# SiftScience/kafka-assigner

Measured on AMD Instinct MI355X. Metric: assignment scenarios/sec at 100k partitions x 1k brokers RF=3, higher is better.
Workload: dtype int32

## Files before the change

kafka-assigner_amd/csrc/kas_order_relax.h:

```cpp
#pragma once

namespace kas {

#define KAS_RELAX_F0_ONE 0x1u
#define KAS_RELAX_F1_ONE 0x10000u
#define KAS_RELAX_F1_MASK 0xffff0000u
#define KAS_RELAX_PAD_WORD 0xfff0fff0u
#define KAS_RELAX_PICK_BITS 0x00010001u

KAS_DEV uint32_t relax_row_word(uint32_t w0, uint32_t w1) { return (KAS_RELAX_F0_ONE << w0) | (KAS_RELAX_F1_ONE << w1); }

#define KAS_RELAX_MAXP 12
struct RelaxPairs {
  uint32_t* slot;
  const uint32_t* row[KAS_RELAX_MAXP];
  uint32_t cell[KAS_RELAX_MAXP];
};

struct RelaxTopic {
  int32_t idx2, idx3;
  uint32_t vp3;
  uint32_t ord2;
};

// ... 11 lines not shown
  }
  return t;
}

KAS_DEV int32_t relax_eval_generic(const uint32_t (&x)[3], const bool (&valid)[3], const int32_t (&rank)[3], int32_t Lp,
                                   const RelaxTopic& t) {
  const int32_t idx_m0 = Lp == 3 ? t.idx3 : (Lp == 2 ? t.idx2 : 0);
  uint32_t best = 0xffffffffu;
#pragma unroll
  for (int k = 0; k < 3; ++k) {
    int32_t vp = idx_m0 + rank[k];
    vp -= vp >= Lp ? Lp : 0;
    const uint32_t key = ((x[k] & 0xffffu) << 8) | ((uint32_t)vp << 2) | (uint32_t)k;
    best = (valid[k] && key < best) ? key : best;
  }
  const int32_t w0 = Lp >= 1 ? (int32_t)(best & 3u) : 0;
  best = 0xffffffffu;
#pragma unroll
  for (int k = 0; k < 3; ++k) {
    const int32_t ord = (Lp == 3 && t.idx2) ? 2 - rank[k] : rank[k];
    const uint32_t key = ((x[k] >> 16) << 8) | ((uint32_t)ord << 2) | (uint32_t)k;
    best = (valid[k] && k != w0 && key < best) ? key : best;
  }
  const int32_t w1 = Lp >= 2 ? (int32_t)(best & 3u) : 0;
  return w0 | (w1 << 2);
}

template <int NP, class Word>
KAS_DEV void relax_exchange(Word* slot, Word* const (&padr)[NP], Word (&padd)[NP], const Word (&nadd)[NP], bool undo) {
  constexpr bool WORD64 = sizeof(Word) == 8;
  if (undo) {
#pragma unroll
    for (int t = 0; t < NP; ++t) {
      if constexpr (WORD64) kasw::lds_sub_u64(padr[t], padd[t]);
      else kasw::lds_sub_u32(padr[t], padd[t]);
    }
  }
  kasw::lockstep();
  Word got[NP];
#pragma unroll
  for (int t = 0; t < NP; ++t) {
    if constexpr (WORD64) got[t] = kasw::lds_add_rtn_u64(padr[t], nadd[t]);
    else got[t] = kasw::lds_add_rtn_u32(padr[t], nadd[t]);
    kasw::lockstep();
    padd[t] = nadd[t];
  }
#pragma unroll
  for (int t = 0; t < NP; ++t) slot[64 * t] = got[t];
  kasw::lockstep();
}

template <int NP>
KAS_DEV void relax_pairs(const RelaxPairs& pp, uint32_t* const (&padr)[NP], uint32_t (&padd)[NP], bool undo) {
  kasw::lockstep();
  uint32_t nadd[NP];
#pragma unroll
  for (int t = 0; t < NP; ++t) nadd[t] = (*pp.row[t] >> pp.cell[t]) & KAS_RELAX_PICK_BITS;
  relax_exchange<NP, uint32_t>(pp.slot, padr, padd, nadd, undo);
}

struct RelaxTags { uint32_t t0[3], t1[3]; };

KAS_DEV RelaxTags relax_tags(const uint32_t (&c)[3], const uint32_t* tagtab) {
  const uint32_t oidx = ((c[0] - c[1]) >> 31) | (((c[0] - c[2]) >> 31) << 1) | (((c[1] - c[2]) >> 31) << 2);
  const uint32_t tw = tagtab[oidx];
  RelaxTags g;
#pragma unroll
  for (int q = 0; q < 3; ++q) { g.t0[q] = (tw >> (4 * q)) & 15u; g.t1[q] = (tw >> (12 + 4 * q)) & 15u; }
  return g;
}

KAS_DEV RelaxTags relax_tags_sorted(const RelaxTopic& t) {
  RelaxTags g;
#pragma unroll
  for (int q = 0; q < 3; ++q) {
    g.t0[q] = ((t.vp3 >> (4 * q)) & 0xcu) | (uint32_t)q;
    g.t1[q] = ((t.ord2 >> (4 * q)) & 0xcu) | (uint32_t)q;
  }
  return g;
}

#ifndef KAS_M32_SORTED_TAGS
#define KAS_M32_SORTED_TAGS(M32) (M32)
#endif
KAS_DEV int32_t relax_eval3(const uint32_t (&x)[3], const RelaxTags& g) {
  const uint32_t k00 = (x[0] << 16) | g.t0[0], k01 = (x[1] << 16) | g.t0[1], k02 = (x[2] << 16) | g.t0[2];
  const uint32_t kmin = k00 < k01 ? (k00 < k02 ? k00 : k02) : (k01 < k02 ? k01 : k02);
  const uint32_t w0 = kmin & 3u;
  const uint32_t k10 = (x[0] & KAS_RELAX_F1_MASK) | g.t1[0], k11 = (x[1] & KAS_RELAX_F1_MASK) | g.t1[1],
                 k12 = (x[2] & KAS_RELAX_F1_MASK) | g.t1[2];
  const uint32_t lo = w0 == 0u ? k11 : k10, hi = w0 == 2u ? k11 : k12;
  const uint32_t w1 = (lo < hi ? lo : hi) & 3u;
  return (int32_t)(w0 | (w1 << 2));
}

template <class Raw>
KAS_DEV void relax_list3(const Raw& raw, int32_t oc, uint32_t (&l)[3], uint32_t* cnt2 = nullptr) {
  const uint32_t w0 = (uint32_t)oc & 3u, w1 = ((uint32_t)oc >> 2) & 3u, w2 = 3u - w0 - w1;
  l[0] = kasw::perm_bytes(raw.w[1], raw.w[0], 0x0c0c0100u + w0 * 0x0202u);
  l[1] = kasw::perm_bytes(raw.w[1], raw.w[0], 0x0c0c0100u + w1 * 0x0202u);
  l[2] = kasw::perm_bytes(raw.w[1], raw.w[0], 0x0c0c0100u + w2 * 0x0202u);
  if (cnt2) kasw::lds_add_u32(cnt2 + l[2], 1u);
}

template <int NB>
struct RelaxPend {
  uint32_t id[NB][3];
  int32_t p;
  int32_t n;
};

template <int W, bool FULLW, bool M32 = false>
KAS_DEV void mid_request(MidRaw<W>& r, const uint16_t* mid, int32_t ow, int32_t p) {
  if constexpr (M32) {
    kasw::gload_u32_async<0>(r.w[0], mid, (uint32_t)p * 4u);
  } else if constexpr (FULLW) {
    const uint32_t off = (uint32_t)p * (uint32_t)(2 * mid_width_of<W>());
    kasw::gload_u32_async<0>(r.w[0], mid, off);
    if constexpr (W == 3) kasw::gload_u16_async<4>(r.w[1], mid, off);
  } else {
    const uint32_t off = (uint32_t)p * (uint32_t)(2 * mid_width(ow));
#pragma unroll
    for (int k = 0; k < W; ++k) kasw::gload_u16_async<0>(r.w[k], mid, off + 2u * (uint32_t)(k < ow ? k : ow - 1));
  }
}
template <int W, bool FULLW, bool M32 = false>
KAS_DEV MidRaw<W> mid_take(const MidRaw<W>& r, int32_t ow, bool active) {
  MidRaw<W> o;
  if constexpr (M32) {
    o.w[0] = active ? r.w[0] : 0xffffffffu;
#pragma unroll
    for (int k = 1; k < W; ++k) o.w[k] = 0xffffffffu;
    return o;
  }
#pragma unroll
  for (int k = 0; k < W; ++k) o.w[k] = (active && (FULLW ? k < (W + 1) / 2 : k < ow)) ? r.w[k] : 0xffffffffu;
  return o;
}

template <int W, bool FULLW, bool M32>
KAS_DEV MidRaw<W> mid_view(const MidRaw<W>& t, int32_t ow) {
  if constexpr (M32) {
    static_assert(W == 3, "dword mid rows: lists 3 wide");
    MidRaw<W> o;
    uint32_t f[3];
    mid32_fields(t.w[0], f);
    if constexpr (FULLW) {
      o.w[0] = f[0] | (f[1] << 16);
      o.w[1] = f[2] | 0xffff0000u;
      o.w[2] = 0xffffffffu;
    } else {
#pragma unroll
      for (int k = 0; k < 3; ++k) o.w[k] = (k < ow && f[k] != KAS_M32_NONE) ? f[k] : 0xffffffffu;
    }
    return o;
  } else {
    return t;
  }
}

template <int NB, bool C16 = false>
KAS_DEV uint64_t relax_flush(RelaxPend<NB>& pend, int32_t* out, uint16_t* out16, uint32_t k) {
  uint64_t d = 0;
#pragma unroll
  for (int b = 0; b < NB; ++b) {
    if (b < pend.n) {
      RowW<3> o;
#pragma unroll
      for (int q = 0; q < 3; ++q) {
        o.v[q] = (int32_t)pend.id[b][q];
        d += kas_digest_cell(k, (uint32_t)(pend.p + 64 * b), (uint32_t)q, o.v[q]);
      }
#if !defined(KAS_TUNE_NO_ROW_STORES)
      if constexpr (C16) {
        uint16_t* row = out16 + (int64_t)(pend.p + 64 * b) * 3;
        store_u32_a2(row, (uint32_t)o.v[0] | ((uint32_t)o.v[1] << 16));
        row[2] = (uint16_t)o.v[2];
      } else {
        *reinterpret_cast<RowW<3>*>(out + (int64_t)(pend.p + 64 * b) * 3) = o;
      }
#endif
    }
  }
  pend.n = 0;
  return d;
// ... 101 lines not shown
  bool aborted = false;
  auto rows_final = [&](int32_t k, int32_t upto) -> bool {
    if constexpr (FS) {
      int32_t idle = 0;
      for (;;) {
        kasw::repoll();
        const uint64_t f = kasw::load_shared_u64_lds(&fs[0]), fk = kasw::load_shared_u64_lds(&fs[1]);
        const int32_t ft = (int32_t)(f >> 32), fr = (int32_t)(uint32_t)f;
        if (kasw::ballot(fk <= (uint64_t)(uint32_t)k) != 0ull) return false;
        if (kasw::ballot(ft > k || (ft == k && fr >= upto)) != 0ull) return true;
        if (watchdog_poll(reinterpret_cast<uint32_t*>(&fs[3]), false, idle)) { stuck = true; return false; }
      }
    }
    return true;
  };
  for (int32_t k = 0; k < sd.topic_count; ++k) {
    const int32_t ti = sd.topic_begin + k;
    if constexpr (FS) {
      if (!rows_final(k, 0)) { aborted = true; break; }
    }
    if (a.topic_results[ti].status != KAS_OK) continue;
    const kas_topic_desc td = a.topics[ti];
    const int32_t P = td.n_partitions, ow = td.out_width;
    if (P <= 0) continue;
    uint64_t dtop = 0;
    int32_t* out = C16 ? nullptr : a.out + td.out_off;
    uint16_t* out16 = C16 ? reinterpret_cast<uint16_t*>(a.out) + td.out_off : nullptr;
    const uint16_t* mid = C16 ? out16 : (M32 ? reinterpret_cast<const uint16_t*>(out + (int64_t)P * ow - P) : mid_base(out, P, ow));
    const RelaxTopic rt = relax_topic(td.name_hash);
    const RelaxTags gsorted = relax_tags_sorted(rt);
    constexpr uint32_t NONE_FROM = M32 ? KAS_M32_NONE : 0x8000u;
    const int32_t nt = (P + 63) >> 6;
    kasw::lockstep();
    if (lane < 8) {
      const int32_t ab = lane & 1, ac = (lane >> 1) & 1, bc = (lane >> 2) & 1;
      const int32_t rank[3] = {(1 - ab) + (1 - ac), ab + (1 - bc), ac + bc};
      uint32_t w = 0u;
#pragma unroll
      for (int q = 0; q < 3; ++q) {
        w |= (((rt.vp3 >> (4 * rank[q])) & 0xcu) | (uint32_t)q) << (4 * q);
        w |= (((rt.ord2 >> (4 * rank[q])) & 0xcu) | (uint32_t)q) << (12 + 4 * q);
      }
      tagtab[lane] = w;
    }
    kasw::lockstep();
    const uint16_t* umid = kasw::uniform_ptr(mid);
    const int32_t* uid = kasw::uniform_ptr(g_node_id);
    auto topic_rows = [&](auto fullw_tag) {
      constexpr bool FULLW = decltype(fullw_tag)::value;
      constexpr int NB = NBT;
      const int32_t vstride = verify_k > 0 ? (nt / verify_k > 0 ? nt / verify_k : 1) : 0;
      const int32_t voff = vstride > 0 ? s % vstride : 0;
      auto row_exists = [&](int32_t t) -> bool { return ((t << 6) + lane) < P; };
      auto request_tile = [&](MidRaw<W>& r, int32_t t) {
        const int32_t pn = (t << 6) + lane;
        mid_request<W, FULLW, M32>(r, umid, ow, pn < P ? pn : 0);
      };
      MidRaw<W> raw[NB], nx[NB];
      RelaxPend<NB> pend;
      pend.n = 0; pend.p = 0;
#pragma unroll
      for (int b = 0; b < NB; ++b) {
#pragma unroll
        for (int q = 0; q < W; ++q) { raw[b].w[q] = 0xffffffffu; nx[b].w[q] = 0xffffffffu; }
#pragma unroll
        for (int q = 0; q < 3; ++q) pend.id[b][q] = 0u;
      }
#pragma unroll
      for (int b = 0; b < NB; ++b) request_tile(nx[b], b);
      kasw::wait_loads();
#pragma unroll
      for (int b = 0; b < NB; ++b) {
#pragma unroll
        for (int q = 0; q < (M32 ? 1 : W); ++q) kasw::arrived(nx[b].w[q]);
        raw[b] = mid_take<W, FULLW, M32>(nx[b], ow, row_exists(b));
      }
#pragma unroll
      for (int b = 0; b < NB; ++b) request_tile(nx[b], NB + b);
      for (int32_t tile = 0; tile < nt;) {
        const int32_t p = (tile << 6) + lane;
        const bool active = p < P;
        const MidRaw<W> ra = mid_view<W, FULLW, M32>(raw[0], ow);
        uint32_t c[3];
        if constexpr (FULLW) {
          c[0] = ra.w[0] & 0xffffu; c[1] = ra.w[0] >> 16; c[2] = W == 3 ? (ra.w[1] & 0xffffu) : KAS_MID_NONE;
        } else {
#pragma unroll
          for (int q = 0; q < 3; ++q) c[q] = q < W ? (ra.w[q] & 0xffffu) : KAS_MID_NONE;
        }
        bool fast = false;
        int32_t step = 1;
        int32_t req_n = 0;
        uint32_t req_l[NB][3];
#pragma unroll
        for (int b = 0; b < NB; ++b)
#pragma unroll
          for (int q = 0; q < 3; ++q) req_l[b][q] = 0u;
        auto usual_step = [&](auto nr_tag) -> bool {
          constexpr int NR = decltype(nr_tag)::value, NP = 3 * NR;
          MidRaw<W> rv[NR];
          uint32_t cc[NR][3];
          rv[0] = ra;
#pragma unroll
          for (int q = 0; q < 3; ++q) cc[0][q] = c[q];
          bool short_row = false;
#pragma unroll
          for (int b = 1; b < NR; ++b) {
            rv[b] = mid_view<W, FULLW, M32>(raw[b], ow);
            cc[b][0] = rv[b].w[0] & 0xffffu; cc[b][1] = rv[b].w[0] >> 16; cc[b][2] = rv[b].w[1] & 0xffffu;
            short_row = short_row || (M32 ? cc[b][2] >= NONE_FROM : ((cc[b][0] | cc[b][1] | cc[b][2]) & 0x8000u) != 0u);
          }
          if constexpr (NR > 1) {
            if (kasw::ballot(short_row) != 0ull) return false;
          }
          n_tiles += NR;
          kasw::lockstep();
#pragma unroll
          for (int b = 0; b < NR; ++b)
#pragma unroll
            for (int q = 0; q < 3; ++q) mine[192 * b + q] = cc[b][q];
          kasw::lockstep();
          uint32_t* padr[NP];
          uint32_t padd[NP];
#pragma unroll
          for (int t = 0; t < NP; ++t) { padr[t] = cnt + pp.slot[64 * t]; padd[t] = 0u; }
          RelaxTags g[NR];
          uint32_t x[NR][3];
#pragma unroll
          for (int b = 0; b < NR; ++b) g[b] = KAS_M32_SORTED_TAGS(M32) ? gsorted : relax_tags(cc[b], tagtab);
#pragma unroll
          for (int b = 0; b < NR; ++b)
#pragma unroll
            for (int q = 0; q < 3; ++q) x[b][q] = cnt[cc[b][q]];
          kasw::lockstep();
          int32_t prev[NR];
#pragma unroll
          for (int b = 0; b < NR; ++b) prev[b] = -1;
#pragma nounroll
          for (int32_t it = 0;; ++it) {
            n_evals += NR;
            if (it > 64 * NR + 2) { stuck = true; break; }
            int32_t oc[NR];
            bool moved = false;
#pragma unroll
            for (int b = 0; b < NR; ++b) { oc[b] = relax_eval3(x[b], g[b]); moved = moved || oc[b] != prev[b]; }
            if (kasw::ballot(moved) == 0ull) break;
#pragma unroll
            for (int b = 0; b < NR; ++b) rbuf[64 * b + lane] = relax_row_word((uint32_t)oc[b] & 3u, (uint32_t)oc[b] >> 2);
            relax_pairs<NP>(pp, padr, padd, it > 0);
#pragma unroll
            for (int b = 0; b < NR; ++b) {
#pragma unroll
              for (int q = 0; q < 3; ++q) x[b][q] = mine[192 * b + q];
              prev[b] = oc[b];
            }
          }
          rows1 += 64u * NR; rows2 += 64u * NR;
          if constexpr (VERIFY) {
            bool sampled = false;
#pragma unroll
            for (int b = 0; b < NR; ++b) sampled = sampled || (vstride > 0 && ((tile + b) % vstride) == voff);
            if (sampled) {
              n_verified += NR;
#pragma unroll
              for (int t = 0; t < NP; ++t) kasw::lds_sub_u32(padr[t], padd[t]);
              kasw::lockstep();
#pragma unroll
              for (int b = 0; b < NR; ++b)
                if (relax_verify_rows(cnt, rv[b].w[0], rv[b].w[1], tagtab, prev[b]) != 0ull) unsound = true;
            }
          }
#pragma unroll
          for (int b = 0; b < NR; ++b) relax_list3(rv[b], prev[b] < 0 ? 4 : prev[b], req_l[b], cnt2);
          req_n = NR;
          step = NR;
          return true;
        };
        bool settled = false;
        if constexpr (W == 3) {
          if (FULLW && ((tile + 1) << 6) <= P)
            fast = M32 ? kasw::ballot(c[2] >= NONE_FROM) == 0ull
                       : kasw::ballot(((c[0] | c[1] | c[2]) & 0x8000u) != 0u) == 0ull;
          if constexpr (NBT > 1) {
            if (fast && ((tile + NBT) << 6) <= P) settled = usual_step(std::integral_constant<int, NBT>{});
          }
          if (!settled && fast) settled = usual_step(std::integral_constant<int, 1>{});
        }
        if (!settled) {
          n_tiles += 1;
          n_slow += 1;
          kasw::lockstep();
#pragma unroll
          for (int q = 0; q < 3; ++q) mine[q] = c[q];
          kasw::lockstep();
          if constexpr (M32) {
#pragma unroll
            for (int q = 0; q < 3; ++q) c[q] = c[q] >= NONE_FROM ? KAS_MID_NONE : c[q];
          }
          uint32_t* padr[3];
          uint32_t padd[3] = {0u, 0u, 0u};
#pragma unroll
          for (int t = 0; t < 3; ++t) {
            const uint32_t n = pp.slot[64 * t];
            padr[t] = cnt + (n < (uint32_t)nmax ? n : (uint32_t)nmax);
          }
          uint32_t x[3];
#pragma unroll
          for (int q = 0; q < 3; ++q) x[q] = cnt[c[q] < (uint32_t)nmax ? c[q] : (uint32_t)nmax];
          kasw::lockstep();
          bool valid[3];
          int32_t rank[3], Lp = 0;
#pragma unroll
          for (int q = 0; q < 3; ++q) { valid[q] = active && (c[q] & 0x8000u) == 0u; Lp += valid[q] ? 1 : 0; }
#pragma unroll
          for (int q = 0; q < 3; ++q) {
            rank[q] = 0;
#pragma unroll
            for (int j = 0; j < 3; ++j) rank[q] += (j != q && valid[j] && c[j] < c[q]) ? 1 : 0;
          }
          rows1 += (uint32_t)kasw::popc(kasw::ballot(Lp >= 1)); rows2 += (uint32_t)kasw::popc(kasw::ballot(Lp >= 2));
          int32_t oc_prev = -1;
          for (int32_t it = 0;; ++it) {
            n_evals += 1;
            if (it > 66) { stuck = true; break; }
            const int32_t oc = relax_eval_generic(x, valid, rank, Lp, rt);
            if (kasw::ballot(oc != oc_prev) == 0ull) break;
            const uint32_t w0 = (uint32_t)oc & 3u, w1 = ((uint32_t)oc >> 2) & 3u;
            rbuf[lane] = (Lp >= 1 ? KAS_RELAX_F0_ONE << w0 : 0u) | (Lp >= 2 ? KAS_RELAX_F1_ONE << w1 : 0u);
            relax_pairs<3>(pp, padr, padd, it > 0);
#pragma unroll
            for (int q = 0; q < 3; ++q) x[q] = mine[q];
            oc_prev = oc;
          }
          if (active && oc_prev >= 0) {
            const int32_t w0 = oc_prev & 3, w1 = (oc_prev >> 2) & 3, w2 = 3 - w0 - w1;
            const int32_t w[3] = {w0, w1, w2};
#pragma unroll
            for (int r = 0; r < W; ++r) {
              if (r < ow) {
                const uint32_t cell = w[r] == 0 ? c[0] : (w[r] == 1 ? c[1] : c[2]);
                const int32_t id = r < Lp ? (C16 ? (int32_t)cell : (LDSIDS ? (int32_t)idt[cell] : g_node_id[cell])) : -1;
                if constexpr (CTX) { if (r == 2 && r < Lp) kasw::lds_add_u32(cnt2 + cell, 1u); }
                if constexpr (C16) out16[(int64_t)p * ow + r] = (uint16_t)id;
                else out[(int64_t)p * ow + r] = id;
                if (r < Lp) dtop += kas_digest_cell((uint32_t)k, (uint32_t)p, (uint32_t)r, id);
              }
            }
          }
        }
        tile += step;
        kasw::wait_loads();
#pragma unroll
        for (int b = 0; b < NB; ++b) {
#pragma unroll
          for (int q = 0; q < (M32 ? 1 : W); ++q) kasw::arrived(nx[b].w[q]);
#pragma unroll
// ... 117 lines not shown
```

kafka-assigner_amd/csrc/kas_solver_body.h:

```cpp
#pragma once
#include <stdint.h>

#include <type_traits>

#include "kas_abi.h"
#include "kas_plan_math.h"
#include "kas_wave.h"

#ifdef KAS_FILL_COUNTERS
#define KAS_COUNT(x) do { (x) += 1; } while (0)
#define KAS_COUNTERS_ON 1
#else
#define KAS_COUNT(x) do { } while (0)
#define KAS_COUNTERS_ON 0
#endif

#ifndef KAS_SPIN_BOUND
#define KAS_SPIN_BOUND (1 << 25)
#endif
#ifndef KAS_WIDE_SPIN_BOUND
#define KAS_WIDE_SPIN_BOUND KAS_SPIN_BOUND
#endif
#ifndef KAS_SPIN_CHECK
#define KAS_SPIN_CHECK 4096
// ... 394 lines not shown
template <int W>
KAS_DEV bool full_rows_of(const TopicView& T) { return T.cw == W && T.ow == W && T.len_arr == nullptr; }

#ifndef KAS_TILES_AHEAD
#define KAS_TILES_AHEAD 4
#endif
template <int W, bool FULL, bool C16, typename Body>
KAS_DEV void for_tiles_impl(const TopicView& T, int32_t tile0, int32_t stride, int32_t t_end, Body body) {
  constexpr int D = KAS_TILES_AHEAD;
  const int lane = kasw::lane();
  int32_t nx[D][W], nlen[D];
#pragma unroll
  for (int d = 0; d < D; ++d) load_row<W, FULL, C16>(T, ((tile0 + d * stride) << 6) + lane, nx[d], nlen[d]);
  for (int32_t tile = tile0; tile < t_end; tile += stride * D) {
    int32_t ids[D][W], len[D];
#pragma unroll
    for (int d = 0; d < D; ++d) {
#pragma unroll
      for (int r = 0; r < W; ++r) ids[d][r] = nx[d][r];
      len[d] = nlen[d];
    }
#pragma unroll
    for (int d = 0; d < D; ++d)
      load_row<W, FULL, C16>(T, ((tile + (D + d) * stride) << 6) + lane, nx[d], nlen[d]);
#pragma unroll
    for (int d = 0; d < D; ++d) {
      const int32_t t = tile + d * stride;
      if (t < t_end) body(t, ids[d], len[d]);
    }
  }
}

template <int W, bool FULL, bool C16, typename Body>
KAS_DEV void for_tile_batches_impl(const TopicView& T, int32_t tile0, int32_t stride, int32_t t_end, Body body) {
  constexpr int D = KAS_TILES_AHEAD;
  const int lane = kasw::lane();
  int32_t nx[D][W], nlen[D];
#pragma unroll
  for (int d = 0; d < D; ++d) load_row<W, FULL, C16>(T, ((tile0 + d * stride) << 6) + lane, nx[d], nlen[d]);
  for (int32_t tile = tile0; tile < t_end; tile += stride * D) {
    int32_t ids[D][W], len[D];
#pragma unroll
    for (int d = 0; d < D; ++d) {
#pragma unroll
      for (int r = 0; r < W; ++r) ids[d][r] = nx[d][r];
      len[d] = (tile + d * stride < t_end) ? nlen[d] : 0;
    }
#pragma unroll
    for (int d = 0; d < D; ++d)
      load_row<W, FULL, C16>(T, ((tile + (D + d) * stride) << 6) + lane, nx[d], nlen[d]);
    body(ids, len);
  }
}

template <int W>
KAS_DEV bool full_rows(const TopicView& T) { return full_rows_of<W>(T); }

template <int W, typename Body>
KAS_DEV void for_tiles(const TopicView& T, int32_t tile0, int32_t stride, int32_t t_end, Body body) {
  if constexpr (W <= 3) if (T.c16) {
    if (full_rows<W>(T)) for_tiles_impl<W, true, true>(T, tile0, stride, t_end, body);
    else for_tiles_impl<W, false, true>(T, tile0, stride, t_end, body);
    return;
  }
  {
    if (full_rows<W>(T)) for_tiles_impl<W, true, false>(T, tile0, stride, t_end, body);
    else for_tiles_impl<W, false, false>(T, tile0, stride, t_end, body);
  }
}

template <int W, typename Body>
KAS_DEV void for_tile_batches(const TopicView& T, int32_t tile0, int32_t stride, int32_t t_end, Body body) {
  if constexpr (W <= 3) if (T.c16) {
    if (full_rows<W>(T)) for_tile_batches_impl<W, true, true>(T, tile0, stride, t_end, body);
    else for_tile_batches_impl<W, false, true>(T, tile0, stride, t_end, body);
    return;
  }
  {
    if (full_rows<W>(T)) for_tile_batches_impl<W, true, false>(T, tile0, stride, t_end, body);
    else for_tile_batches_impl<W, false, false>(T, tile0, stride, t_end, body);
  }
}

template <int W>
KAS_DEV void p3_rows(const LdsView& L, const TopicView& T, int32_t p, int32_t len,
                     const int32_t (&ids)[W], const int32_t (&idx)[W], uint32_t accbits,
                     int32_t& need, int32_t& hc, int32_t (&hrack)[W], int32_t& moved_r,
                     int32_t& moved_p, const int32_t* racks = nullptr, bool inplace = false) {
  const bool active = p < T.P;
  int32_t hold[W];
#pragma unroll
  for (int k = 0; k < W; ++k) { hold[k] = -1; hrack[k] = -1; }
  hc = 0;
#pragma unroll
  for (int r = 0; r < W; ++r) {
    const bool acc = (accbits >> r) & 1u;
    const int32_t n = idx[r] >= 0 ? idx[r] : 0;
    const int32_t rk = racks ? racks[r] : (int32_t)lds_rack(L, n);
#pragma unroll
    for (int k = 0; k < W; ++k) {
      const bool here = acc && hc == k;
      hold[k] = here ? n : hold[k];
      hrack[k] = here ? rk : hrack[k];
    }
    hc += acc ? 1 : 0;
  }
  const bool in_parts = active && (T.inp_arr ? T.inp_arr[p] != 0 : true);
  need = in_parts ? (T.rf - hc > 0 ? T.rf - hc : 0) : 0;
#if defined(KAS_TUNE_NO_ORPHANS)
  {
#pragma unroll
    for (int k = 0; k < W; ++k) hold[k] = (k >= hc && k < T.rf) ? (int32_t)((uint32_t)(p * 7 + k * 131) % (uint32_t)T.N) : hold[k];
    need = 0;
  }
#endif
  bool same = inplace && KAS_IXROWS_SKIP_SAME;
#pragma unroll
  for (int k = 0; k < W; ++k) same = same && hold[k] == idx[k];
#if defined(KAS_TUNE_NO_MID_STORES)
  if (false) {
#else
  if (active && !same) {
#endif
    if (W == 3 && T.m32) {
      if constexpr (W == 3) reinterpret_cast<uint32_t*>(T.mid)[p] = mid32_pack(hold[0], hold[1], hold[2]);
    } else if (T.ow == W) {
      uint16_t* row = T.mid + (int64_t)p * mid_width_of<W>();
#pragma unroll
      for (int k = 0; k < W / 2; ++k)
        store_u32_a2(row + 2 * k, ((uint32_t)hold[2 * k] & 0xffffu) | (((uint32_t)hold[2 * k + 1] & 0xffffu) << 16));
      if constexpr (W & 1) row[W - 1] = (uint16_t)hold[W - 1];
    } else {
#pragma unroll
      for (int k = 0; k < W; ++k)
        if (k < mid_width(T.ow)) T.mid[(int64_t)p * mid_width(T.ow) + k] = (uint16_t)hold[k];
    }
  }
  uint32_t kept_else = 0;
#pragma unroll
  for (int r = 0; r < W; ++r)
#pragma unroll
    for (int r2 = 0; r2 < W; ++r2)
      kept_else |= (((accbits >> r2) & 1u) != 0u && ids[r2] == ids[r]) ? (1u << r) : 0u;
  const uint32_t present = len >= W ? ((1u << W) - 1u) : ((1u << len) - 1u);
  const bool dropped = (present & ~accbits & ~kept_else) != 0u;
  moved_r += need;
  moved_p += (active && (dropped || need > 0)) ? 1 : 0;
}

template <int W>
KAS_DEV void ring_push(const LdsView& L, int32_t p, int32_t need, int32_t hc,
                       const int32_t (&hrack)[W], int32_t& ring_count) {
  const bool orphan = need > 0;
  const uint64_t om = kasw::ballot(orphan);
  if (orphan) {
    const int32_t slot = ring_count + kasw::count_below(om);
    L.ring_p[slot] = p;
    L.ring_meta[slot] = need | (hc << 8);
#pragma unroll
    for (int k = 0; k < W; ++k) L.ring_rack[k * KAS_RING_CAP + slot] = (int16_t)hrack[k];
  }
  ring_count += kasw::popc(om);
  kasw::lockstep();
}

template <int W>
KAS_DEV int32_t drain_ring(const LdsView& L, const TopicView& T, int32_t min_fill, int32_t live_count,
                           int32_t& head, int32_t& ring_count, int64_t (&st)[8]) {
  const int lane = kasw::lane();
  while (ring_count >= min_fill && ring_count > 0) {
    const int32_t n_win = ring_count < 64 ? ring_count : 64;
    const int32_t fl = p4_window<W>(L, n_win, T.cap, live_count, head, T.mid, mid_width(T.ow), st, T.m32);
    if (fl >= 0) return L.ring_p[fl];
    const int32_t rest = ring_count - n_win;
    int32_t tp = 0, tm = 0; int32_t tr[W];
#pragma unroll
    for (int k = 0; k < W; ++k) tr[k] = 0;
    if (lane < rest) {
      tp = L.ring_p[64 + lane]; tm = L.ring_meta[64 + lane];
#pragma unroll
      for (int k = 0; k < W; ++k) tr[k] = L.ring_rack[k * KAS_RING_CAP + 64 + lane];
    }
    kasw::lockstep();
    if (lane < rest) {
      L.ring_p[lane] = tp; L.ring_meta[lane] = tm;
#pragma unroll
      for (int k = 0; k < W; ++k) L.ring_rack[k * KAS_RING_CAP + lane] = (int16_t)tr[k];
    }
    ring_count = rest;
    kasw::lockstep();
  }
  return -1;
}

template <int W>
KAS_DEV_COLD void fill_generic_sweeps(const LdsView& L, const TopicView& T, const NodeMap& nm,
                                 uint64_t* accmask, int64_t (&st)[8]) {
  const int lane = kasw::lane();
  const int32_t cap = T.cap, nt = T.nt;
  if (T.P <= 0 || T.cw <= 0) return;
  for (int32_t r = 0; r < T.cw; ++r) {
    for_tiles<W>(T, 0, 1, nt, [&](int32_t tile, const int32_t (&ids)[W], int32_t len) {
      int32_t n = -1;
      if (r < len) n = node_lookup(L, nm, sel<W>(ids, r));
      bool elig = n >= 0;
      const int32_t rk = elig ? (int32_t)lds_rack(L, n) : -1;
#pragma unroll
      for (int r2 = 0; r2 < W - 1; ++r2) {
        if (r2 < r) {
          const uint64_t aw = kasw::load_shared_u64(accmask + (int64_t)r2 * nt + tile);
          if (elig && ((aw >> lane) & 1ull)) {
            const int32_t n2 = node_lookup(L, nm, ids[r2]);
            if ((int32_t)lds_rack(L, n2) == rk) elig = false;
          }
        }
      }
      const bool took = elig && lds_load(L, n) < cap;
      kasw::lockstep();
      if (took) kasw::lds_atomic_add(&lds_load(L, n), 1);
      kasw::lockstep();
      bool accepted = took;
      uint64_t todo = kasw::ballot(took && lds_load(L, n) > cap);
      if (todo != 0) {
        KAS_COUNT(st[7]);
        while (todo != 0) {
          const int leader = kasw::first_lane(todo);
// ... 166 lines not shown
        tot[r] += h[w][r];
      }
    int32_t cum = 0, rs = W, q = 0;
#pragma unroll
    for (int r = 0; r < W; ++r) {
      const int32_t c = tot[r];
      const bool sat = rs == W && c > T.cap - cum;
      q = sat ? T.cap - cum : q;
      cum = rs == W ? (sat ? T.cap : cum + c) : cum;
      rs = sat ? r : rs;
    }
    lds_load(L, n) = cum;
    lds_qrs(L, n) = (int32_t)(((uint32_t)rs << 28) | (uint32_t)q);
    int32_t rem = q;
#pragma unroll
    for (int w = 0; w < NW; ++w) {
      int32_t c = 0;
#pragma unroll
      for (int r = 0; r < W; ++r) c = rs == r ? h[w][r] : c;
      L.x[n * BW + w] = rem;
      rem -= c;
    }
  }
}

template <int W, int NW>
KAS_DEV void fill_quota(const LdsView& L, const TopicView& T, int32_t tid) {
  const int32_t N = T.N;
  for (int32_t n = tid; n < N; n += 64 * NW) {
    int32_t cum = 0, rs = W, q = 0;
#pragma unroll
    for (int r = 0; r < W; ++r) {
      const int32_t c = L.x[r * N + n];
      const bool sat = rs == W && c > T.cap - cum;
      q = sat ? T.cap - cum : q;
      cum = rs == W ? (sat ? T.cap : cum + c) : cum;
      rs = sat ? r : rs;
    }
    lds_load(L, n) = cum;
    lds_qrs(L, n) = (int32_t)(((uint32_t)rs << 28) | (uint32_t)q);
#pragma unroll
    for (int w = 0; w < NW; ++w) L.x[w * N + n] = NW == 1 ? q : 0;
  }
}

template <int W, int NW, bool DIRECT>
KAS_DEV void fill_chunk_count(const LdsView& L, const TopicView& T, const NodeMap& nm, int32_t wave) {
  constexpr int D = KAS_TILES_AHEAD;
  const int32_t N = T.N;
  const int32_t t0 = chunk_begin<NW>(T.nt, wave), t1 = chunk_begin<NW>(T.nt, wave + 1);
  int32_t* qc = L.x + wave * N;
  for_tile_batches<W>(T, t0, 1, t1, [&](const int32_t (&ids)[D][W], const int32_t (&len)[D]) {
    int32_t idx[D][W], rs[D][W];
#pragma unroll
    for (int d = 0; d < D; ++d)
#pragma unroll
      for (int r = 0; r < W; ++r) idx[d][r] = r < len[d] ? node_lookup_as<DIRECT>(L, nm, ids[d][r]) : -1;
#pragma unroll
    for (int d = 0; d < D; ++d)
#pragma unroll
      for (int r = 0; r < W; ++r)
        rs[d][r] = idx[d][r] >= 0 ? (int32_t)((uint32_t)lds_qrs(L, idx[d][r]) >> 28) : -1;
#pragma unroll
    for (int d = 0; d < D; ++d)
#pragma unroll
      for (int r = 0; r < W; ++r) if (rs[d][r] == r) kasw::lds_atomic_add(&qc[idx[d][r]], 1);
  });
}

template <int NW>
KAS_DEV void fill_chunk_prefix(const LdsView& L, const TopicView& T, int32_t tid) {
  const int32_t N = T.N;
  for (int32_t n = tid; n < N; n += 64 * NW) {
    int32_t rem = lds_qrs(L, n) & 0x0fffffff;
#pragma unroll
    for (int w = 0; w < NW; ++w) {
      const int32_t c = L.x[w * N + n];
      L.x[w * N + n] = rem;
      rem -= c;
    }
  }
}

template <int W, bool DIRECT, int QS, bool RTN = false, bool INPLACE = false>
KAS_DEV int32_t fill_pass_b_range(const LdsView& L, const TopicView& T, const NodeMap& nm, int32_t t0, int32_t t1,
                                  int32_t* qc, int32_t& moved_r, int32_t& moved_p, int64_t (&st)[8]) {
  const int lane = kasw::lane();
  int32_t* olist = T.orph + ((int64_t)t0 << 6);
  int32_t ocount = 0;
  for_tiles<W>(T, t0, 1, t1, [&](int32_t tile, const int32_t (&ids)[W], int32_t len) {
    const int32_t p = (tile << 6) + lane;
    int32_t idx[W], nn[W], before[W];
    uint32_t sure = 0, counting = 0;
#pragma unroll
    for (int r = 0; r < W; ++r) {
      int32_t rs;
      if constexpr (RTN && DIRECT) {
        const uint32_t d = (uint32_t)ids[r] - (uint32_t)nm.min_id;
        const uint32_t raw = (r < len && d < nm.range) ? (uint32_t)(uint16_t)L.idmap[d] : 0xffffu;
        idx[r] = raw != 0xffffu ? (int32_t)(raw & 0x3fffu) : -1;
        rs = (int32_t)(raw >> 14);
      } else {
        idx[r] = r < len ? node_lookup_as<DIRECT>(L, nm, ids[r]) : -1;
        rs = (int32_t)((uint32_t)lds_qrs(L, idx[r] >= 0 ? idx[r] : 0) >> 28);
      }
      nn[r] = idx[r] >= 0 ? idx[r] : 0;
      sure |= (idx[r] >= 0 && r < rs) ? (1u << r) : 0u;
      counting |= (idx[r] >= 0 && r == rs) ? (1u << r) : 0u;
      if constexpr (!RTN) before[r] = qc[nn[r] * QS];
    }
    uint32_t accbits = sure;
    if constexpr (RTN) {
      if (kasw::ballot(counting != 0u) != 0) {
#pragma unroll
        for (int r = 0; r < W; ++r) {
          kasw::lockstep();
          int32_t left = 0;
          if ((counting >> r) & 1u) left = (int32_t)kasw::lds_add_rtn_u32((uint32_t*)&qc[nn[r] * QS], 0xffffffffu);
          accbits |= (((counting >> r) & 1u) && left > 0) ? (1u << r) : 0u;
        }
        kasw::lockstep();
      }
    } else if (kasw::ballot(counting != 0u) != 0) {
      kasw::lockstep();
#pragma unroll
      for (int r = 0; r < W; ++r) if ((counting >> r) & 1u) kasw::lds_atomic_add(&qc[nn[r] * QS], -1);
      kasw::lockstep();
      uint32_t contested = 0;
#pragma unroll
      for (int r = 0; r < W; ++r) {
        const int32_t after = qc[nn[r] * QS];
        const bool cnt = (counting >> r) & 1u;
        accbits |= (cnt && after >= 0) ? (1u << r) : 0u;
        contested |= (cnt && before[r] > 0 && after < 0) ? (1u << r) : 0u;
      }
      uint64_t todo = kasw::ballot(contested != 0u);
      if (todo != 0) {
        KAS_COUNT(st[7]);
        while (todo != 0) {
          const int leader = kasw::first_lane(todo);
          int32_t mine_t = -1;
#pragma unroll
          for (int r = W - 1; r >= 0; --r) mine_t = ((contested >> r) & 1u) ? nn[r] : mine_t;
          const int32_t t = kasw::shfl(mine_t, leader);
          uint32_t hit = 0;
#pragma unroll
          for (int r = 0; r < W; ++r) hit |= (((counting >> r) & 1u) && nn[r] == t) ? (1u << r) : 0u;
          const uint64_t same = kasw::ballot(hit != 0u);
          const int32_t rank = kasw::count_below(same);
#pragma unroll
          for (int r = 0; r < W; ++r)
            accbits |= (((hit >> r) & 1u) && rank < before[r]) ? (1u << r) : 0u;
          contested &= ~hit;
          todo = kasw::ballot(contested != 0u);
        }
      }
    }
    int32_t need, hc, hrack[W];
    p3_rows<W>(L, T, p, len, ids, idx, accbits, need, hc, hrack, moved_r, moved_p, nullptr, INPLACE);
    const uint64_t om = kasw::ballot(need > 0);
    if (need > 0) olist[ocount + kasw::count_below(om)] = p;
    ocount += kasw::popc(om);
  });
  return ocount;
}
template <int W, int NW, bool DIRECT, bool FUSED = false, bool RTN = false, bool INPLACE = false>
KAS_DEV int32_t fill_pass_b(const LdsView& L, const TopicView& T, const NodeMap& nm, int32_t wave,
                            int32_t& moved_r, int32_t& moved_p, int64_t (&st)[8]) {
  const int32_t t0 = chunk_begin<NW>(T.nt, wave), t1 = chunk_begin<NW>(T.nt, wave + 1);
  constexpr int QS = FUSED ? fused_block_words<W, NW>() : 1;
  int32_t* qc = FUSED ? L.x + wave : L.x + wave * T.N;
  return fill_pass_b_range<W, DIRECT, QS, RTN, INPLACE>(L, T, nm, t0, t1, qc, moved_r, moved_p, st);
}

KAS_DEV TopicView topic_view(const KasLaunch& a, const kas_topic_desc& td, int32_t N, int m32c = -1) {
  TopicView T;
  T.c16 = cells16(a);
  T.cur = topic_cur(a, td);
  T.len_arr = td.cur_len_off >= 0 ? a.aux + td.cur_len_off : nullptr;
  T.inp_arr = td.in_partitions_off >= 0 ? a.aux + td.in_partitions_off : nullptr;
  T.pid_arr = td.part_id_off >= 0 ? a.aux + td.part_id_off : nullptr;
  T.P = td.n_partitions; T.cw = td.cur_width; T.rf = td.rf; T.ow = td.out_width;
  T.hash = td.name_hash; T.nt = (T.P + 63) >> 6; T.N = N;
  T.mid = topic_mid(a, td);
  T.m32 = m32c < 0 ? mid32(a) : (m32c != 0);
  return T;
}

KAS_DEV bool nodes_bad(const int32_t* ids, const int32_t* racks, int32_t N, int32_t first, int32_t stride) {
  bool bad = false;
  for (int32_t i = first; i < N; i += stride) {
    const int32_t id = ids[i];
    const int32_t prev = i > 0 ? ids[i - 1] : -1;
    const int32_t rk = racks[i];
    bad = bad || id <= prev || rk < 0 || rk > 32767;
  }
  return bad;
}

KAS_DEV NodeMap node_map_of(const int32_t* ids, int32_t N, int32_t idmap_entries, bool checked) {
  NodeMap nm;
  nm.n = N; nm.min_id = 0; nm.range = 0u;
  if (N > 0) {
    const int64_t lo = ids[0], hi = ids[N - 1];
    const int64_t range = hi - lo + 1;
    nm.min_id = (int32_t)lo;
    if ((checked || range >= 1) && range <= (int64_t)idmap_entries) nm.range = (uint32_t)range;
  }
  return nm;
}

KAS_DEV LdsView lds_view(const KasLds& lay, unsigned char* lds_raw) {
  LdsView L;
  L.x = (int32_t*)(lds_raw + lay.off_x);
  L.load = (int32_t*)(lds_raw + lay.off_load);
  L.qrs = (int32_t*)(lds_raw + lay.off_qrs);
  L.rack = (int16_t*)(lds_raw + lay.off_rack);
  L.live = (int16_t*)(lds_raw + lay.off_live);
  L.ns = 1; L.rs = 1;
  L.idmap = (int16_t*)(lds_raw + lay.off_idmap);
  L.ids = (int32_t*)(lds_raw + lay.off_ids);
  L.ring_p = (int32_t*)(lds_raw + lay.off_ring);
  L.ring_meta = L.ring_p + KAS_RING_CAP;
  L.ring_rack = (int16_t*)(L.ring_meta + KAS_RING_CAP);
  L.ctl = (int32_t*)(lds_raw + lay.off_ctl);
  return L;
}

KAS_DEV void put_topic_result(const KasLaunch& a, int32_t ti, const TopicOutcome& o) {
  kas_topic_result tr;
  tr.status = o.status; tr.fail_partition = o.fail_partition;
  tr.moved_replicas = o.moved_replicas; tr.moved_partitions = o.moved_partitions;
  a.topic_results[ti] = tr;
}
KAS_DEV void put_scenario_result(const KasLaunch& a, int32_t s, int32_t status, int32_t fail_topic, int32_t fail_partition,
                                 int32_t moved_r, int32_t moved_p) {
  kas_scenario_result sr;
  sr.status = status; sr.fail_topic = fail_topic; sr.fail_partition = fail_partition;
  sr.moved_replicas = moved_r; sr.moved_partitions = moved_p; sr.reserved = 0;
  sr.digest = 0;
  a.scenario_results[s] = sr;
}

}

#include "kas_first_fit.h"

namespace kas {

template <int W>
KAS_DEV void pick_row(const int32_t (&c)[W][W], int32_t Lp, bool valid, const int32_t (&idxm)[W + 1],
                      int32_t (&pos)[W], int32_t (&cnt_r)[W]) {
  uint32_t alive = valid ? ((1u << Lp) - 1u) : 0u;
#pragma unroll
  for (int r = 0; r < W; ++r) {
// ... 64 lines not shown
  const int tid = kasw::tid();
  for (int32_t i = tid; i < N; i += 64 * NW) p4s[KAS_P4S_HEAD + i] = lds_load(L, i);
  if (tid == 0) { p4s[0] = 1; p4s[1] = cap; }
  if (tid < NW) p4s[2 + tid] = L.ctl[KAS_CTL_OC + tid];
  publish_moved(L, moved_r, moved_p);
  kasw::sync();
  phase_tick(st, 3, tmark);
  res.moved_replicas = L.ctl[KAS_CTL_MOVED_R];
  res.moved_partitions = L.ctl[KAS_CTL_MOVED_P];
}

#define KAS_TOPIC_NEEDS_FULL_FILL (-1000)
template <int W, int NW, bool SLIM = false, int M32C = -1>
KAS_DEV TopicOutcome fill_topic(const KasLaunch& a, const kas_topic_desc& td, const LdsView& L,
                                const NodeMap& nm, const int32_t* g_node_id, const int32_t* g_node_rack,
                                uint64_t* accmask, int32_t* orph, int32_t* p4s, int64_t (&st)[8]) {
  constexpr int NT = 64 * NW;
  const int lane = kasw::lane();
  const int tid = kasw::tid();
  const int32_t wave = kasw::wave_id();
  const uint64_t lt = kasw::lanemask_lt();
  const int32_t N = nm.n;
  TopicView T = topic_view(a, td, N, M32C);
  T.orph = orph;
  const int32_t P = T.P, hash = T.hash;

  TopicOutcome res;
  res.status = KAS_OK; res.fail_partition = -1;
  res.moved_replicas = 0; res.moved_partitions = 0;

  int64_t tmark = kasw::clock_ticks();
  int32_t n_in = P;
  if (T.inp_arr) {
    int32_t c = 0;
    for (int32_t p = lane; p < P; p += 64) c += T.inp_arr[p] != 0 ? 1 : 0;
    n_in = kasw::wave_sum(c);
  }
  T.cap = max_replicas_per_node(N, n_in, T.rf);
  const int32_t cap = T.cap;

  const bool try_fast = P > 0 && T.cw > 0 && !(a.flags & KAS_FLAG_GENERIC_FILL) && cap >= 0 && cap < (1 << 28);
  const bool fused = W <= 3 && NW > 1 && (a.flags & KAS_FLAG_FUSED_HIST) != 0u;
  if (fused) {
    constexpr int BW = fused_block_words<(W <= 3 ? W : 3), (NW > 1 ? NW : 2)>();
    for (int32_t i = tid; i < N; i += NT) {
#pragma unroll
      for (int k = 0; k < BW - 1; ++k) L.x[i * BW + k] = 0;
      lds_rack(L, i) = (int16_t)g_node_rack[i];
    }
  } else {
    for (int32_t i = tid; i < N; i += NT) {
      lds_load(L, i) = 0;
      lds_rack(L, i) = (int16_t)g_node_rack[i];
    }
    if (try_fast)
      for (int32_t i = tid; i < N * W; i += NT) L.x[i] = 0;
  }
  if (nm.range != 0u) {
    for (uint32_t i = (uint32_t)tid; i < nm.range; i += (uint32_t)NT) L.idmap[i] = (int16_t)-1;
  } else {
    for (int32_t i = tid; i < N; i += NT) L.ids[i] = g_node_id[i];
  }
  first_fit_reset_ctl(L, tid);
  kasw::sync();
  if (nm.range != 0u)
    for (int32_t i = tid; i < N; i += NT) L.idmap[(uint32_t)g_node_id[i] - (uint32_t)nm.min_id] = (int16_t)i;
  kasw::sync();
  phase_tick(st, 0, tmark);

  if constexpr (SLIM) {
    static_assert(W <= 3 && NW > 1, "the slim fill is the per-chunk-histogram form");
    const bool mine = try_fast && fused && !T.c16 && (a.flags & KAS_FLAG_LANE_ORDER) != 0u && !(a.flags & KAS_FLAG_INDEX_ROWS) &&
                      nm.range != 0u && p4s != nullptr;
    if (!mine) { res.status = KAS_TOPIC_NEEDS_FULL_FILL; return res; }
    const bool viol = fill_pass_a_fused<W, NW, true>(L, T, nm, wave);
    if (kasw::ballot(viol) != 0 && lane == 0) L.ctl[KAS_CTL_VIOL] = 1;
    kasw::sync();
    if (L.ctl[KAS_CTL_VIOL] != 0) { res.status = KAS_TOPIC_NEEDS_FULL_FILL; return res; }
    fill_quota_fused<W, NW>(L, T, tid);
    kasw::sync();
    phase_tick(st, 1, tmark);
    pack_idmap_with_rstar<NT, true>(L, N, g_node_id, nm.min_id);
    int32_t moved_r = 0, moved_p = 0;
    const int32_t oc = fill_pass_b<W, NW, true, true, true>(L, T, nm, wave, moved_r, moved_p, st);
    if (lane == 0) L.ctl[KAS_CTL_OC + wave] = oc;
    kasw::sync();
    phase_tick(st, 2, tmark);
    if (java_abs_mod(hash, N) < 0) { res.status = KAS_FAIL_HASH_INDEX; return res; }
    hand_over_to_p4<NW>(L, N, cap, p4s, moved_r, moved_p, res, st, tmark);
    return res;
  } else {
  bool fast = false;
  const bool ixrows = W <= 3 && NW > 1 && try_fast && fused && !T.c16 && (a.flags & KAS_FLAG_INDEX_ROWS) != 0u &&
                      (a.flags & KAS_FLAG_LANE_ORDER) != 0u && nm.range != 0u && full_rows_of<W>(T) && N < 0x3fff;
  if (try_fast) {
    bool viol;
    if constexpr (W <= 3 && NW > 1) {
      if (fused) viol = ixrows ? fill_pass_a_fused<W, NW, true, false, true>(L, T, nm, wave)
                        : (T.c16 && nm.range != 0u && nm.min_id == 0) ? fill_pass_a_fused<W, NW, true, true>(L, T, nm, wave)
                        : (nm.range != 0u ? fill_pass_a_fused<W, NW, true>(L, T, nm, wave) : fill_pass_a_fused<W, NW, false>(L, T, nm, wave));
      else viol = nm.range != 0u ? fill_pass_a<W, NW, true>(L, T, nm, wave) : fill_pass_a<W, NW, false>(L, T, nm, wave);
    } else {
      viol = nm.range != 0u ? fill_pass_a<W, NW, true>(L, T, nm, wave) : fill_pass_a<W, NW, false>(L, T, nm, wave);
    }
    if (kasw::ballot(viol) != 0 && lane == 0) L.ctl[KAS_CTL_VIOL] = 1;
    kasw::sync();
    fast = L.ctl[KAS_CTL_VIOL] == 0;
    if (!fast) {
      for (int32_t i = tid; i < N; i += NT) lds_load(L, i) = 0;
      kasw::sync();
    }
  }
  int32_t moved_r = 0, moved_p = 0;
  if (fast) {
    int32_t oc = 0;
    bool done = false;
    if constexpr (W <= 3 && NW > 1) {
      if (fused) {
        fill_quota_fused<W, NW>(L, T, tid);
        kasw::sync();
        phase_tick(st, 1, tmark);
        if (ixrows) {
          st[6] += 1;
          pack_idmap_with_rstar<NT, false>(L, N, nullptr, 0);
          TopicView T2 = T;
          T2.c16 = true;
          T2.cur = reinterpret_cast<const int32_t*>(T.mid);
          NodeMap nm2;
          nm2.n = N; nm2.min_id = 0; nm2.range = (uint32_t)N;
          oc = fill_pass_b<W, NW, true, true, true, true>(L, T2, nm2, wave, moved_r, moved_p, st);
        }
        else if (a.flags & KAS_FLAG_LANE_ORDER) {
          if (nm.range != 0u) {
            pack_idmap_with_rstar<NT, true>(L, N, g_node_id, nm.min_id);
            oc = fill_pass_b<W, NW, true, true, true>(L, T, nm, wave, moved_r, moved_p, st);
          } else {
            oc = fill_pass_b<W, NW, false, true, true>(L, T, nm, wave, moved_r, moved_p, st);
          }
        }
        else
          oc = nm.range != 0u ? fill_pass_b<W, NW, true, true>(L, T, nm, wave, moved_r, moved_p, st)
                              : fill_pass_b<W, NW, false, true>(L, T, nm, wave, moved_r, moved_p, st);
        done = true;
      }
    }
    if (!done) {
      fill_quota<W, NW>(L, T, tid);
      kasw::sync();
      if (NW > 1) {
        if (nm.range != 0u) fill_chunk_count<W, NW, true>(L, T, nm, wave);
        else fill_chunk_count<W, NW, false>(L, T, nm, wave);
        kasw::sync();
        fill_chunk_prefix<NW>(L, T, tid);
        kasw::sync();
      }
      phase_tick(st, 1, tmark);
      oc = nm.range != 0u ? fill_pass_b<W, NW, true>(L, T, nm, wave, moved_r, moved_p, st)
                          : fill_pass_b<W, NW, false>(L, T, nm, wave, moved_r, moved_p, st);
    }
    if (lane == 0) L.ctl[KAS_CTL_OC + wave] = oc;
  } else if (wave == 0) {
    fill_generic_sweeps<W>(L, T, nm, accmask, st);
    phase_tick(st, 1, tmark);
  }
  kasw::sync();
  phase_tick(st, 2, tmark);

// ... 1164 lines not shown
```

Baseline: 661,700.

## Pick relax lists from unpacked mid32 fields and simplify sorted p3 row output

In the relax loop, dword mid rows are now unpacked with mid32_fields, and the three ordered replica lists are chosen with bitfield-insert selects on those fields instead of byte permutes on raw words. That path also skips the cnt2 LDS increment. In the slim fill, when rows are 3 wide and use dword mids, p3_rows takes a SORTED/DISTINCT path: it fills held slots directly, counts them with popcount, always stores the packed row, and skips the duplicate-id scan and the same-row check. The aim is fewer ALU and LDS operations per row. It relies on rows being sorted and distinct, and on cnt2 not being needed on that path.

```diff
diff --git a/kafka-assigner_amd/csrc/kas_order_relax.h b/kafka-assigner_amd/csrc/kas_order_relax.h
--- a/kafka-assigner_amd/csrc/kas_order_relax.h
+++ b/kafka-assigner_amd/csrc/kas_order_relax.h
@@ -117,6 +117,9 @@
 
 #ifndef KAS_M32_SORTED_TAGS
 #define KAS_M32_SORTED_TAGS(M32) (M32)
+#endif
+#ifndef KAS_RELAX_PICK_FIELDS
+#define KAS_RELAX_PICK_FIELDS 1
 #endif
 KAS_DEV int32_t relax_eval3(const uint32_t (&x)[3], const RelaxTags& g) {
   const uint32_t k00 = (x[0] << 16) | g.t0[0], k01 = (x[1] << 16) | g.t0[1], k02 = (x[2] << 16) | g.t0[2];
@@ -136,6 +139,23 @@
   l[1] = kasw::perm_bytes(raw.w[1], raw.w[0], 0x0c0c0100u + w1 * 0x0202u);
   l[2] = kasw::perm_bytes(raw.w[1], raw.w[0], 0x0c0c0100u + w2 * 0x0202u);
   if (cnt2) kasw::lds_add_u32(cnt2 + l[2], 1u);
+}
+
+KAS_DEV uint32_t relax_bits_select(uint32_t m, uint32_t a, uint32_t b) {
+#if defined(__HIP_DEVICE_COMPILE__)
+  uint32_t r;
+  asm("v_bfi_b32 %0, %1, %2, %3" : "=v"(r) : "v"(m), "v"(a), "v"(b));
+  return r;
+#else
+  return (a & m) | (b & ~m);
+#endif
+}
+KAS_DEV void relax_pick3(const uint32_t (&v)[3], int32_t oc, uint32_t (&l)[3]) {
+  const uint32_t m01 = (uint32_t)((int32_t)((uint32_t)oc << 31) >> 31), m02 = (uint32_t)((int32_t)((uint32_t)oc << 30) >> 31);
+  const uint32_t m11 = (uint32_t)((int32_t)((uint32_t)oc << 29) >> 31), m12 = (uint32_t)((int32_t)((uint32_t)oc << 28) >> 31);
+  l[0] = relax_bits_select(m02, v[2], relax_bits_select(m01, v[1], v[0]));
+  l[1] = relax_bits_select(m12, v[2], relax_bits_select(m11, v[1], v[0]));
+  l[2] = v[0] ^ v[1] ^ v[2] ^ l[0] ^ l[1];
 }
 
 template <int NB>
@@ -403,7 +423,9 @@
         const bool active = p < P;
         const MidRaw<W> ra = mid_view<W, FULLW, M32>(raw[0], ow);
         uint32_t c[3];
-        if constexpr (FULLW) {
+        if constexpr (M32 && FULLW) {
+          mid32_fields(raw[0].w[0], c);
+        } else if constexpr (FULLW) {
           c[0] = ra.w[0] & 0xffffu; c[1] = ra.w[0] >> 16; c[2] = W == 3 ? (ra.w[1] & 0xffffu) : KAS_MID_NONE;
         } else {
 #pragma unroll
@@ -428,7 +450,8 @@
 #pragma unroll
           for (int b = 1; b < NR; ++b) {
             rv[b] = mid_view<W, FULLW, M32>(raw[b], ow);
-            cc[b][0] = rv[b].w[0] & 0xffffu; cc[b][1] = rv[b].w[0] >> 16; cc[b][2] = rv[b].w[1] & 0xffffu;
+            if constexpr (M32) mid32_fields(raw[b].w[0], cc[b]);
+            else { cc[b][0] = rv[b].w[0] & 0xffffu; cc[b][1] = rv[b].w[0] >> 16; cc[b][2] = rv[b].w[1] & 0xffffu; }
             short_row = short_row || (M32 ? cc[b][2] >= NONE_FROM : ((cc[b][0] | cc[b][1] | cc[b][2]) & 0x8000u) != 0u);
           }
           if constexpr (NR > 1) {
@@ -492,7 +515,11 @@
             }
           }
 #pragma unroll
-          for (int b = 0; b < NR; ++b) relax_list3(rv[b], prev[b] < 0 ? 4 : prev[b], req_l[b], cnt2);
+          for (int b = 0; b < NR; ++b) {
+            const int32_t ocf = prev[b] < 0 ? 4 : prev[b];
+            if constexpr (M32 && KAS_RELAX_PICK_FIELDS) relax_pick3(cc[b], ocf, req_l[b]);
+            else relax_list3(rv[b], ocf, req_l[b], cnt2);
+          }
           req_n = NR;
           step = NR;
           return true;
diff --git a/kafka-assigner_amd/csrc/kas_solver_body.h b/kafka-assigner_amd/csrc/kas_solver_body.h
--- a/kafka-assigner_amd/csrc/kas_solver_body.h
+++ b/kafka-assigner_amd/csrc/kas_solver_body.h
@@ -500,16 +500,25 @@
   }
 }
 
-template <int W>
+#ifndef KAS_P3_SORTED_OUT
+#define KAS_P3_SORTED_OUT 1
+#endif
+template <int W, bool SORTED_OUT = false, bool DISTINCT = false>
 KAS_DEV void p3_rows(const LdsView& L, const TopicView& T, int32_t p, int32_t len,
                      const int32_t (&ids)[W], const int32_t (&idx)[W], uint32_t accbits,
                      int32_t& need, int32_t& hc, int32_t (&hrack)[W], int32_t& moved_r,
                      int32_t& moved_p, const int32_t* racks = nullptr, bool inplace = false) {
+  static_assert(!SORTED_OUT || W == 3, "dword mid rows: lists 3 wide");
   const bool active = p < T.P;
   int32_t hold[W];
 #pragma unroll
   for (int k = 0; k < W; ++k) { hold[k] = -1; hrack[k] = -1; }
   hc = 0;
+  if constexpr (SORTED_OUT) {
+#pragma unroll
+    for (int r = 0; r < W; ++r) hold[r] = ((accbits >> r) & 1u) ? (idx[r] >= 0 ? idx[r] : 0) : -1;
+    hc = kasw::popc((uint64_t)(accbits & ((1u << W) - 1u)));
+  } else {
 #pragma unroll
   for (int r = 0; r < W; ++r) {
     const bool acc = (accbits >> r) & 1u;
@@ -523,6 +532,7 @@
     }
     hc += acc ? 1 : 0;
   }
+  }
   const bool in_parts = active && (T.inp_arr ? T.inp_arr[p] != 0 : true);
   need = in_parts ? (T.rf - hc > 0 ? T.rf - hc : 0) : 0;
 #if defined(KAS_TUNE_NO_ORPHANS)
@@ -532,7 +542,7 @@
     need = 0;
   }
 #endif
-  bool same = inplace && KAS_IXROWS_SKIP_SAME;
+  bool same = !SORTED_OUT && inplace && KAS_IXROWS_SKIP_SAME;
 #pragma unroll
   for (int k = 0; k < W; ++k) same = same && hold[k] == idx[k];
 #if defined(KAS_TUNE_NO_MID_STORES)
@@ -540,7 +550,7 @@
 #else
   if (active && !same) {
 #endif
-    if (W == 3 && T.m32) {
+    if (SORTED_OUT || (W == 3 && T.m32)) {
       if constexpr (W == 3) reinterpret_cast<uint32_t*>(T.mid)[p] = mid32_pack(hold[0], hold[1], hold[2]);
     } else if (T.ow == W) {
       uint16_t* row = T.mid + (int64_t)p * mid_width_of<W>();
@@ -555,11 +565,15 @@
     }
   }
   uint32_t kept_else = 0;
+  if constexpr (DISTINCT) {
+    kept_else = accbits;
+  } else {
 #pragma unroll
   for (int r = 0; r < W; ++r)
 #pragma unroll
     for (int r2 = 0; r2 < W; ++r2)
       kept_else |= (((accbits >> r2) & 1u) != 0u && ids[r2] == ids[r]) ? (1u << r) : 0u;
+  }
   const uint32_t present = len >= W ? ((1u << W) - 1u) : ((1u << len) - 1u);
   const bool dropped = (present & ~accbits & ~kept_else) != 0u;
   moved_r += need;
@@ -892,7 +906,7 @@
   }
 }
 
-template <int W, bool DIRECT, int QS, bool RTN = false, bool INPLACE = false>
+template <int W, bool DIRECT, int QS, bool RTN = false, bool INPLACE = false, bool SORTED = false>
 KAS_DEV int32_t fill_pass_b_range(const LdsView& L, const TopicView& T, const NodeMap& nm, int32_t t0, int32_t t1,
                                   int32_t* qc, int32_t& moved_r, int32_t& moved_p, int64_t (&st)[8]) {
   const int lane = kasw::lane();
@@ -967,20 +981,20 @@
       }
     }
     int32_t need, hc, hrack[W];
-    p3_rows<W>(L, T, p, len, ids, idx, accbits, need, hc, hrack, moved_r, moved_p, nullptr, INPLACE);
+    p3_rows<W, SORTED, SORTED>(L, T, p, len, ids, idx, accbits, need, hc, hrack, moved_r, moved_p, nullptr, INPLACE);
     const uint64_t om = kasw::ballot(need > 0);
     if (need > 0) olist[ocount + kasw::count_below(om)] = p;
     ocount += kasw::popc(om);
   });
   return ocount;
 }
-template <int W, int NW, bool DIRECT, bool FUSED = false, bool RTN = false, bool INPLACE = false>
+template <int W, int NW, bool DIRECT, bool FUSED = false, bool RTN = false, bool INPLACE = false, bool SORTED = false>
 KAS_DEV int32_t fill_pass_b(const LdsView& L, const TopicView& T, const NodeMap& nm, int32_t wave,
                             int32_t& moved_r, int32_t& moved_p, int64_t (&st)[8]) {
   const int32_t t0 = chunk_begin<NW>(T.nt, wave), t1 = chunk_begin<NW>(T.nt, wave + 1);
   constexpr int QS = FUSED ? fused_block_words<W, NW>() : 1;
   int32_t* qc = FUSED ? L.x + wave : L.x + wave * T.N;
-  return fill_pass_b_range<W, DIRECT, QS, RTN, INPLACE>(L, T, nm, t0, t1, qc, moved_r, moved_p, st);
+  return fill_pass_b_range<W, DIRECT, QS, RTN, INPLACE, SORTED>(L, T, nm, t0, t1, qc, moved_r, moved_p, st);
 }
 
 KAS_DEV TopicView topic_view(const KasLaunch& a, const kas_topic_desc& td, int32_t N, int m32c = -1) {
@@ -1211,7 +1225,7 @@
     phase_tick(st, 1, tmark);
     pack_idmap_with_rstar<NT, true>(L, N, g_node_id, nm.min_id);
     int32_t moved_r = 0, moved_p = 0;
-    const int32_t oc = fill_pass_b<W, NW, true, true, true>(L, T, nm, wave, moved_r, moved_p, st);
+    const int32_t oc = fill_pass_b<W, NW, true, true, true, false, W == 3 && M32C == 1 && KAS_P3_SORTED_OUT>(L, T, nm, wave, moved_r, moved_p, st);
     if (lane == 0) L.ctl[KAS_CTL_OC + wave] = oc;
     kasw::sync();
     phase_tick(st, 2, tmark);
```

Result: faster. 676,300, median of 6 (+2.2%).
